# mahyarnajibi/SNIPER

Hardware: AMD Instinct MI355X
Metric: train chips/sec (512x512, R101) (higher is better)
Workload: dtype f16

## Files before the change

include/sniper_hip.h:

```cpp
#ifndef SNIPER_HIP_H
#define SNIPER_HIP_H

#include <stddef.h>
#include <stdint.h>

#ifdef __cplusplus
extern "C" {
#endif

typedef void *sn_stream_t;

enum { SN_OK = 0, SN_ERR_ARG = 1, SN_ERR_HIP = 2, SN_ERR_WORKSPACE = 3, SN_ERR_UNSUPPORTED = 4 };

int sn_version(void);
const char *sn_last_error(void);
int sn_debug_option(const char *name, int value);

int sn_iou_f64(const double *d_boxes, int N, const double *d_query, int K, double *d_out, int mode, sn_stream_t stream);

int sn_chips_num_candidates(int width, int height, int chipsize, int stride);
size_t sn_chips_workspace_bytes(int total_cand, int max_boxes_per_unit);
int sn_chips_generate_batch(const float *d_boxes, const int32_t *d_box_off, const int32_t *d_meta, const int32_t *d_perm,
                            const int32_t *d_cand_off, int U, int max_boxes_per_unit, void *d_mask_ws, float *d_out_chips,
                            int32_t *d_out_ids, int32_t *d_out_count, sn_stream_t stream);
// ... 74 lines not shown
                       int KH, int KWP, int stride, void *ws, size_t ws_bytes, sn_stream_t stream);
int sn_conv_dgrad(const void *dy, const void *wt, const void *accumulate, void *dx, int N, int H, int W, int Cin,
                  int dx_pix_stride, int Cout, int dy_pix_stride, int acc_pix_stride, int KH, int KW, int stride, int pad, int dil,
                  int out_f32, sn_stream_t stream);
int sn_conv_dgrad_by_class(int on);
int sn_conv_dgrad_bn_blocks(int N, int H, int W, int Cin, int dx_pix_stride, int Cout, int dy_pix_stride, int acc_pix_stride, int KH,
                            int KW, int stride, int pad, int dil);
int sn_conv_dgrad_bn(const void *dy, const void *wt, const void *accumulate, void *dx, int N, int H, int W, int Cin, int dx_pix_stride,
                     int Cout, int dy_pix_stride, int acc_pix_stride, int KH, int KW, int stride, int pad, int dil, const void *bn_x,
                     int bn_x_pix_stride, const float *bn_scale, const float *bn_shift, const float *bn_mean, int bn_act,
                     float *partials, sn_stream_t stream);
size_t sn_conv_wgrad_workspace_bytes(int N, int H, int W, int Cin, int x_pix_stride, int Cout, int dy_pix_stride, int KH, int KW,
                                     int stride, int pad, int dil);
int sn_conv_wgrad(const void *dy, const void *x, float *dw, int N, int H, int W, int Cin, int x_pix_stride, int Cout,
                  int dy_pix_stride, int KH, int KW, int stride, int pad, int dil, void *ws, size_t ws_bytes, sn_stream_t stream);
typedef struct sn_wgrad_desc {
  const void *dy, *x;
  float *dw;
  int N, H, W, Cin, x_pix_stride, Cout, dy_pix_stride, KH, KW, stride, pad, dil;
} sn_wgrad_desc;
size_t sn_conv_wgrad_batch_workspace_bytes(const sn_wgrad_desc *descs, int n);
int sn_conv_wgrad_batch(const sn_wgrad_desc *descs, int n, void *ws, size_t ws_bytes, sn_stream_t stream);
int sn_conv_wgrad_impl(int impl, int job_steps);
int sn_conv_wgrad_trace(void *buf);
int sn_conv_trace(void *buf);
size_t sn_bias_grad_workspace_bytes(long rows, int C);
int sn_bias_grad(const void *dy, float *db, long rows, int C, int ld, int dtype, void *ws, size_t ws_bytes, sn_stream_t stream);

int sn_pack_stem_input(const float *x_nchw, void *out, int N, int C, int H, int W, int Hp, int Wp, int pad_t, int pad_l,
                       const float *scale, const float *shift, sn_stream_t stream);

size_t sn_bn_workspace_bytes(int M, int C);
int sn_bn_stats(const void *x, int M, int C, int ps, void *ws, sn_stream_t stream);
int sn_bn_finalize(const void *ws, int M, int C, float eps, float momentum, const float *gamma, const float *beta,
                   float *run_mean, float *run_var, float *scale, float *shift, float *save_mean, float *save_invstd,
                   sn_stream_t stream);
int sn_bn_finalize_blocks(const float *partials, int nblk, int M, int C, float eps, float momentum, const float *gamma,
                          const float *beta, float *run_mean, float *run_var, float *scale, float *shift, float *save_mean,
                          float *save_invstd, sn_stream_t stream);
int sn_bn_global_scale_shift(const float *gamma, const float *beta, const float *mean, const float *var, int C, float eps,
                             float *scale, float *shift, sn_stream_t stream);
int sn_bn_apply(const void *x, void *y, int M, int C, int ps_in, int ps_out, const float *scale, const float *shift, int relu,
                sn_stream_t stream);
int sn_bn_apply_blocks(const float *partials, int nblk, const void *x, void *y, int M, int C, int ps_in, int ps_out, float eps,
                       float momentum, const float *gamma, const float *beta, float *run_mean, float *run_var, float *scale,
                       float *shift, float *save_mean, float *save_invstd, int relu, sn_stream_t stream);
// ... 110 lines not shown
```

sniper_amd/csrc/conv.hip:

```cpp
#include <algorithm>
#include <atomic>

#include "conv_common.h"

#include <stdlib.h>

__device__ __forceinline__ int swz(int row, int chunk) { return chunk ^ ((0x78 >> (2 * ((row >> 2) & 3))) & 3); }

template <int BM, int BN, bool DGRAD>
__global__ __launch_bounds__(256) void conv_igemm_kernel(const ConvParams p) {
  constexpr int BK = 32;
  constexpr int WM = BM / 2, WN = BN / 2;
  constexpr int MI = WM / 16, NI = WN / 16;
  constexpr int AR = BM / 64, BR = BN / 64;
  __shared__ __attribute__((aligned(16))) half_t sA[2][BM * BK];
  __shared__ __attribute__((aligned(16))) half_t sB[2][BN * BK];

  const int tid = threadIdx.x, lane = tid & 63, wave = tid >> 6;
  const int wm = wave >> 1, wn = wave & 1;
  const int m0 = blockIdx.x * BM, n0 = blockIdx.y * BN;
  const int chunk = tid & 3, lrow = tid >> 2;

  int a_base[AR], a_h[AR], a_w[AR];
  bool a_ok[AR];
// ... 624 lines not shown
  p.KH = KH; p.KW = KW; p.stride = stride; p.pad = pad; p.dil = dil;
  SN_REQUIRE(N > 0 && H > 0 && W > 0 && Cin > 0 && Cout > 0, "sn_conv_wgrad: bad dims");
  WgradPlan q = wgrad_plan(N, H, W, Cin, Cout, KH, KW, stride, pad, dil);
  p.Ho = q.Ho; p.Wo = q.Wo;
  SN_REQUIRE(p.Ho > 0 && p.Wo > 0, "sn_conv_wgrad: bad dims");
  const size_t n = (size_t)Cout * q.taps * Cin;
  p.slab = nullptr;
  p.slab_stride = n;
  if (q.splits > 1) {
    if (ws && ws_bytes >= sizeof(float) * (size_t)q.splits * n && ((uintptr_t)ws % 16) == 0) p.slab = (float *)ws;
    else { q.splits = 1; q.units_per_split = q.nunits; }
  }
  p.units_per_split = q.units_per_split;
  hipLaunchKernelGGL(conv_wgrad_kernel, dim3(wgrad_grid(p, q.gx, q.gy, q.taps * q.splits)), dim3(256), 0, s, p);
  SN_CHECK_LAUNCH();
  if (p.slab) {
    hipLaunchKernelGGL(wgrad_reduce_kernel, dim3(sn_blocks((long)(n / 4), 4096)), dim3(256), 0, s, (const float *)p.slab, q.splits, n, dw);
    SN_CHECK_LAUNCH();
  }
  return SN_OK;
}

static std::atomic<int> g_wgrad_na{0};
static std::atomic<int> g_wgrad_impl{1};
SN_EXPORT int sn_conv_wgrad_impl(int impl, int job_steps) {
  SN_REQUIRE((impl == 0 || impl == 1) && job_steps >= 0, "sn_conv_wgrad_impl: impl in {0, 1}, job_steps >= 0");
  SN_REQUIRE(job_steps / 100000 <= 2, "sn_conv_wgrad_impl: bad tile selector");
  g_wgrad_impl.store(impl, std::memory_order_relaxed);
  g_wgrad_na.store(job_steps / 100000, std::memory_order_relaxed);
  wgrad_ps_set_job_steps(job_steps % 100000);
  return SN_OK;
}

SN_EXPORT int sn_conv_trace(void *buf) {
  conv_dma_set_trace(static_cast<unsigned long long *>(buf));
  return SN_OK;
}

SN_EXPORT int sn_conv_wgrad_trace(void *buf) {
  wgrad_ps_set_trace(static_cast<unsigned long long *>(buf));
  return SN_OK;
}

static bool wgrad_desc_params(const sn_wgrad_desc &d, WgradParams &p) {
  p.dy = (const half_t *)d.dy; p.x = (const half_t *)d.x; p.dw = d.dw;
  p.N = d.N; p.H = d.H; p.W = d.W; p.Cin = d.Cin; p.Cout = d.Cout; p.dy_ps = d.dy_pix_stride; p.x_ps = d.x_pix_stride;
  p.KH = d.KH; p.KW = d.KW; p.stride = d.stride; p.pad = d.pad; p.dil = d.dil;
  if (d.N <= 0 || d.H <= 0 || d.W <= 0 || d.Cin <= 0 || d.Cout <= 0 || d.KH <= 0 || d.KW <= 0 || d.stride <= 0 || d.dil <= 0) return false;
  p.Ho = sn_conv_out(d.H, d.KH, d.stride, d.pad, d.dil);
  p.Wo = sn_conv_out(d.W, d.KW, d.stride, d.pad, d.dil);
  p.slab = nullptr; p.slab_stride = 0; p.units_per_split = 0;
  return p.Ho > 0 && p.Wo > 0;
}

static int wgrad_batch_run(const sn_wgrad_desc *descs, int n, void *ws, size_t ws_bytes, hipStream_t s, bool launch, size_t *need) {
  size_t off = 0;
  WgradParams chunk[kWgradMaxProblems];
  int nc = 0, na = 1;
  auto flush = [&]() -> int {
    if (!nc) return SN_OK;
    WgradBatch tab;
    char *base = ws ? static_cast<char *>(ws) + off : nullptr;
    size_t bytes = wgrad_ps_plan(chunk, nc, tab, base, true, na);
    if (launch) {
      if (bytes && !(ws && off + bytes <= ws_bytes && ((uintptr_t)base % 16) == 0)) bytes = wgrad_ps_plan(chunk, nc, tab, nullptr, false, na);
      if (int rc = wgrad_ps_launch(tab, s, na)) return rc;
    }
    off += bytes;
    nc = 0;
    return SN_OK;
  };
  for (int i = 0; i < n; ++i) {
    WgradParams p;
    SN_REQUIRE(wgrad_desc_params(descs[i], p), "sn_conv_wgrad_batch: bad dims in problem %d", i);
    if (launch) SN_REQUIRE(descs[i].dy && descs[i].x && descs[i].dw, "sn_conv_wgrad_batch: null pointer in problem %d", i);
  }
  auto fill = [](long j) { return j <= 0 ? 0.0 : (double)j / (256.0 * (double)((j + 255) / 256)); };
  for (int pass = 2; pass >= 1; --pass) {
    na = pass;
    long jobs = 0;
    for (int i = 0; i < n; ++i) {
      const sn_wgrad_desc &d = descs[i];
      WgradParams p;
      wgrad_desc_params(d, p);
      if (!(g_wgrad_impl.load(std::memory_order_relaxed) == 1 && wgrad_ps_ok(p))) continue;
      const int na_forced = g_wgrad_na.load(std::memory_order_relaxed);
      const int want = na_forced ? na_forced : (p.Cout > 128 ? 2 : 1);
      if (want != pass) continue;
      const bool flat = p.KH == 1 && p.KW == 1 && p.stride == 1 && p.pad == 0;
      const long steps = flat ? sn_div_up(sn_div_up(p.N * p.H * p.W, 32), 2) : sn_div_up(p.N * p.Ho * sn_div_up(p.Wo, 32), 2);
      const long j = (long)sn_div_up(p.Cout, 128 * na) * sn_div_up(p.Cin, 128) * p.KH * p.KW * ((steps + 399) / 400);
      if (nc && jobs >= 200 && fill(jobs) >= 0.93 && fill(jobs + j) < fill(jobs) - 0.02) {
        if (int rc = flush()) return rc;
        jobs = 0;
      }
      chunk[nc++] = p;
      jobs += j;
      if (nc == kWgradMaxProblems) {
        if (int rc = flush()) return rc;
        jobs = 0;
      }
    }
    if (int rc = flush()) return rc;
  }
  for (int i = 0; i < n; ++i) {
    const sn_wgrad_desc &d = descs[i];
    WgradParams p;
    wgrad_desc_params(d, p);
    if (g_wgrad_impl.load(std::memory_order_relaxed) == 1 && wgrad_ps_ok(p)) continue;
    const size_t bytes = wgrad_legacy_workspace_bytes(d.N, d.H, d.W, d.Cin, d.x_pix_stride, d.Cout, d.dy_pix_stride, d.KH, d.KW, d.stride, d.pad, d.dil);
    if (launch) {
      char *base = ws ? static_cast<char *>(ws) + off : nullptr;
      const size_t have = ws && off + bytes <= ws_bytes ? bytes : 0;
      if (int rc = wgrad_legacy(d.dy, d.x, d.dw, d.N, d.H, d.W, d.Cin, d.x_pix_stride, d.Cout, d.dy_pix_stride, d.KH, d.KW, d.stride, d.pad,
                                d.dil, have ? base : nullptr, have, s))
        return rc;
    }
    off += bytes;
  }
  if (need) *need = off;
  return SN_OK;
}

SN_EXPORT size_t sn_conv_wgrad_batch_workspace_bytes(const sn_wgrad_desc *descs, int n) {
  size_t need = 0;
  if (!descs || n <= 0 || wgrad_batch_run(descs, n, nullptr, 0, nullptr, false, &need)) return 0;
  return need;
}

SN_EXPORT int sn_conv_wgrad_batch(const sn_wgrad_desc *descs, int n, void *ws, size_t ws_bytes, sn_stream_t stream) {
  SN_REQUIRE(descs && n > 0, "sn_conv_wgrad_batch: empty table");
  return wgrad_batch_run(descs, n, ws, ws_bytes, sn_stream(stream), true, nullptr);
}

SN_EXPORT size_t sn_conv_wgrad_workspace_bytes(int N, int H, int W, int Cin, int x_pix_stride, int Cout, int dy_pix_stride, int KH,
                                               int KW, int stride, int pad, int dil) {
  const sn_wgrad_desc d = {nullptr, nullptr, nullptr, N, H, W, Cin, x_pix_stride, Cout, dy_pix_stride, KH, KW, stride, pad, dil};
  return sn_conv_wgrad_batch_workspace_bytes(&d, 1);
}

SN_EXPORT int sn_conv_wgrad(const void *dy, const void *x, float *dw, int N, int H, int W, int Cin, int x_pix_stride,
                            int Cout, int dy_pix_stride, int KH, int KW, int stride, int pad, int dil, void *ws,
                            size_t ws_bytes, sn_stream_t stream) {
// ... 49 lines not shown
```

sniper_amd/csrc/conv_common.h:

```cpp
#pragma once
#include <atomic>
#include "common.h"

struct ConvParams {
  const half_t *x;
  const half_t *w;
  void *y;
  const float *bias;
  const half_t *res;
  int N, H, W;
  int Cin, in_ps;
  int Ho, Wo;
  int Nout, out_ps, res_ps;
  int KH, KW, stride, pad, dil;
  int M;
  int relu, out_f32;
  unsigned x_bytes, w_bytes;
  const half_t *bn_x = nullptr;
  const float *bn_scale = nullptr, *bn_shift = nullptr, *bn_mean = nullptr;
  int bn_x_ps = 0, bn_act = 0;
  unsigned fda_mul = 1, fda_sh = 0, fdb_mul = 1, fdb_sh = 0;
  int rows_img = 1, row_len = 1;
  int cls = 0, cls_mc = 0;
  int ksplit = 1, ksplit_grid = 0;
// ... 70 lines not shown
  return true;
}
static inline unsigned wgrad_grid(WgradParams &p, int gx, int gy, int gz) {
  p.gx = gx; p.gy = gy; p.gz = gz;
  p.per_xcd = (gx * gy * gz + 7) / 8;
  return 8u * (unsigned)p.per_xcd;
}

struct WgradProblem {
  const half_t *dy, *x;
  float *dw, *slab;
  size_t slab_stride;
  int N, H, W, Ho, Wo, Cin, Cout, dy_ps, x_ps, KH, KW, stride, pad, dil;
  int gx, gy, taps, splits, units_per_split, cpr, nunits, item0;
};
constexpr int kWgradMaxProblems = 24;
struct WgradBatch {
  int n, total_items, per_xcd, reserved;
  int xcd_start[9];
  int reserved2;
  unsigned long long *trace;
  WgradProblem p[kWgradMaxProblems];
};
bool wgrad_ps_ok(const WgradParams &p);
size_t wgrad_ps_plan(const WgradParams *ps, int n, WgradBatch &tab, void *ws, bool allow_split, int na);
int wgrad_ps_launch(const WgradBatch &tab, hipStream_t s, int na);
void wgrad_ps_set_job_steps(int steps);
void wgrad_ps_set_trace(unsigned long long *buf);
```

sniper_amd/csrc/conv_wgrad_ps.hip:

```cpp
#include "conv_common.h"
#include <type_traits>

namespace {

constexpr int kTrSecond = 16 * 128;

constexpr unsigned kPoison = 0x80000000u;

constexpr int kTile = 64 * 128;

template <int S, int NA, int MI, bool TRACE>
__global__ __launch_bounds__(64 * (16 * NA / MI + 4)) void wgrad_ps_kernel(const WgradBatch tab) {
  constexpr int NI = 4, NC = 16 * NA / MI, L = 4 * (NA + 1);
  constexpr int kStage = (NA + 1) * kTile;
  static_assert((S - 1) * L < 64, "vmcnt is a 6-bit counter");
  __shared__ __attribute__((aligned(1024))) half_t lds[S * kStage];
  const int tid = threadIdx.x, lane = tid & 63;
  const int wave = __builtin_amdgcn_readfirstlane(tid >> 6);
  const unsigned long long t_entry = TRACE ? __builtin_amdgcn_s_memtime() : 0;
  const int b = blockIdx.x;
  const int item = tab.xcd_start[b & 7] + (b >> 3);
  if (item >= tab.xcd_start[(b & 7) + 1]) return;
  int pi = 0;
  while (pi + 1 < tab.n && item >= tab.p[pi + 1].item0) ++pi;
  const WgradProblem &P = tab.p[pi];
  const int gx = P.gx, taps = P.taps, tiles = gx * P.gy;
  int r = item - P.item0;
  const int bz = r / tiles;
  r -= bz * tiles;
  const int by = r / gx, bx = r - by * gx;
  const int split = bz / taps, tap = bz - split * taps;
  const int kh = tap / P.KW, kw = tap - kh * P.KW;
  const int co0 = bx * (128 * NA), ci0 = by * 128;
  const int Cout = P.Cout, Cin = P.Cin;
  const int u_begin = split * P.units_per_split, u_end = min(P.nunits, u_begin + P.units_per_split);
  const int nk = u_end > u_begin ? (u_end - u_begin + 1) >> 1 : 0;

  if (wave >= NC) {
    const int h = (wave - NC) >> 1, sub = (wave - NC) & 1;
    const int r4 = lane >> 4, slot = lane & 15;
    const unsigned dy_ps_b = (unsigned)P.dy_ps * 2u, x_ps_b = (unsigned)P.x_ps * 2u;
    const int stride = P.stride, Wo = P.Wo, Ho = P.Ho, H = P.H, W = P.W, cpr = P.cpr;
    const int row_shift = kh * P.dil - P.pad;
    unsigned a_base[NA][2], b_base[2];
#pragma unroll
    for (int o = 0; o < 2; ++o) {
      const int gc = ((((slot >> 1) ^ ((o << 2) | r4)) << 1) | (slot & 1));
      const int ur = 16 * sub + r4;
#pragma unroll
      for (int ta = 0; ta < NA; ++ta) {
// ... 32 lines not shown
          it_xc = 0;
          ++it_r;
          if (++it_oy == Ho) { it_oy = 0; ++it_img; }
        }
    };
#pragma unroll
    for (int s = 0; s < S - 1; ++s)
      if (s < nk) issue(s);
    int nxt = S - 1;
    unsigned long long c_wait = 0, c_bar = 0, c_issue = 0, t0 = 0, t1 = 0, t2 = 0;
    for (int t = 0; t < nk; ++t) {
      if (TRACE) t0 = __builtin_amdgcn_s_memtime();
      const int young = min(S - 2, nk - 1 - t);
      if (S > 3 && young >= 2) wait_vmcnt<(S > 3 ? 2 : 0) * L>();
      else if (S > 2 && young == 1) wait_vmcnt<(S > 2 ? 1 : 0) * L>();
      else wait_vmcnt<0>();
      if (TRACE) t1 = __builtin_amdgcn_s_memtime();
      __builtin_amdgcn_s_barrier();
      if (TRACE) t2 = __builtin_amdgcn_s_memtime();
      if (t + S - 1 < nk) issue(nxt);
      nxt = nxt + 1 == S ? 0 : nxt + 1;
      if (TRACE) { c_wait += t1 - t0; c_bar += t2 - t1; c_issue += __builtin_amdgcn_s_memtime() - t2; }
    }
    if (TRACE && wave == NC && lane == 0 && tab.trace) {
      unsigned long long *o = tab.trace + (size_t)item * 8;
      o[4] = c_wait; o[5] = c_bar; o[6] = c_issue;
    }
    return;
  }

  const int wm = wave >> 1, wn = wave & 1;
  const int fr = lane & 15, fq = lane >> 4;
  const int row0 = fq * 4 + (fr >> 2), q7 = row0 & 7;
  int a_off[MI], b_off[NI];
#pragma unroll
  for (int i = 0; i < MI; ++i) {
    const int rb = wm * MI + i;
    a_off[i] = (rb >> 3) * kTile + row0 * 128 + ((((rb & 7) ^ q7) << 4) | ((fr & 3) << 2));
  }
#pragma unroll
  for (int jn = 0; jn < NI; ++jn) b_off[jn] = row0 * 128 + ((((wn * 4 + jn) ^ q7) << 4) | ((fr & 3) << 2));
  floatx4 acc[MI][NI];
#pragma unroll
  for (int i = 0; i < MI; ++i)
#pragma unroll
    for (int jn = 0; jn < NI; ++jn) acc[i][jn] = floatx4{0.f, 0.f, 0.f, 0.f};
  unsigned long long c_bar = 0, tb = 0;
  const unsigned long long t_loop = TRACE ? __builtin_amdgcn_s_memtime() : 0;
// ... 29 lines not shown
  };
  if (nk > 0) {
    step_barrier();
    read(0, 0, fa0, fb0);
    __builtin_amdgcn_sched_barrier(0);
  }
  int cur = 0, nxt = 1;
  for (int t = 0; t + 1 < nk; ++t) {
    mma(fa0, fb0);
    read(cur, 1, fa1, fb1);
    interleave();
    step_barrier();
    __builtin_amdgcn_sched_barrier(0);
    mma(fa1, fb1);
    read(nxt, 0, fa0, fb0);
    interleave();
    cur = nxt;
    nxt = nxt + 1 == S ? 0 : nxt + 1;
  }
  if (nk > 0) {
    mma(fa0, fb0);
    read(cur, 1, fa1, fb1);
    interleave();
    mma(fa1, fb1);
  }
  const unsigned long long t_epi = TRACE ? __builtin_amdgcn_s_memtime() : 0;
  float *dst = P.slab ? P.slab + (size_t)split * P.slab_stride : P.dw;
  const bool to_slab = P.slab != nullptr;
  if ((Cin & 3) == 0) {
#pragma unroll
    for (int i0 = 0; i0 < MI; i0 += 4) {
      float *q[4][NI];
      bool ok[4][NI];
#pragma unroll
      for (int i = 0; i < 4; ++i)
#pragma unroll
        for (int jn = 0; jn < NI; ++jn) {
          const int co = co0 + (wm * MI + i0 + i) * 16 + fr, ci = ci0 + wn * 64 + jn * 16 + fq * 4;
          ok[i][jn] = co < Cout && ci < Cin;
          q[i][jn] = dst + ((size_t)co * taps + tap) * Cin + ci;
        }
      if (!to_slab) {
        float4 o[4][NI];
#pragma unroll
        for (int i = 0; i < 4; ++i)
#pragma unroll
          for (int jn = 0; jn < NI; ++jn) o[i][jn] = ok[i][jn] ? *reinterpret_cast<const float4 *>(q[i][jn]) : make_float4(0.f, 0.f, 0.f, 0.f);
#pragma unroll
// ... 5 lines not shown
          }
      }
#pragma unroll
      for (int i = 0; i < 4; ++i)
#pragma unroll
        for (int jn = 0; jn < NI; ++jn)
          if (ok[i][jn]) *reinterpret_cast<float4 *>(q[i][jn]) = make_float4(acc[i0 + i][jn][0], acc[i0 + i][jn][1], acc[i0 + i][jn][2], acc[i0 + i][jn][3]);
    }
  } else {
#pragma unroll
    for (int i = 0; i < MI; ++i) {
      const int co = co0 + (wm * MI + i) * 16 + fr;
      if (co >= Cout) continue;
#pragma unroll
      for (int jn = 0; jn < NI; ++jn) {
        const int ci = ci0 + wn * 64 + jn * 16 + fq * 4;
        float *qq = dst + ((size_t)co * taps + tap) * Cin + ci;
#pragma unroll
        for (int rr = 0; rr < 4; ++rr)
          if (ci + rr < Cin) qq[rr] = to_slab ? acc[i][jn][rr] : qq[rr] + acc[i][jn][rr];
      }
    }
  }
  if (TRACE && wave == 0 && lane == 0 && tab.trace) {
    asm volatile("s_waitcnt vmcnt(0)" ::: "memory");
    const unsigned long long t_end = __builtin_amdgcn_s_memtime();
    unsigned long long *o = tab.trace + (size_t)item * 8;
    o[0] = t_end - t_entry; o[1] = t_epi - t_loop; o[2] = c_bar; o[3] = t_end - t_epi; o[7] = (unsigned long long)nk;
  }
}

constexpr int kReduceBlocksMax = 1024;
__device__ __forceinline__ int reduce_blocks_of(const WgradProblem &q) {
  if (!q.slab) return 0;
  const long b = (long)((q.slab_stride / 4 + 255) / 256);
  return (int)(b < 1 ? 1 : (b > kReduceBlocksMax ? kReduceBlocksMax : b));
}
__global__ __launch_bounds__(256) void wgrad_reduce_batch_kernel(const WgradBatch tab) {
  int b = blockIdx.x, pi = 0, nb = 0;
  for (; pi < tab.n; ++pi) {
    nb = reduce_blocks_of(tab.p[pi]);
    if (b < nb) break;
    b -= nb;
  }
  if (pi >= tab.n) return;
  const WgradProblem &q = tab.p[pi];
  const float *__restrict__ slab = q.slab;
  float *__restrict__ dw = q.dw;
  const size_t n = q.slab_stride, n4 = n >> 2;
  const int splits = q.splits;
  for (size_t i = (size_t)b * 256 + threadIdx.x; i < n4; i += (size_t)nb * 256) {
    float4 a = reinterpret_cast<const float4 *>(dw)[i];
    int s = 0;
    for (; s + 8 <= splits; s += 8) {
      float4 v[8];
#pragma unroll
      for (int k = 0; k < 8; ++k) v[k] = reinterpret_cast<const float4 *>(slab + (size_t)(s + k) * n)[i];
#pragma unroll
      for (int k = 0; k < 8; ++k) { a.x += v[k].x; a.y += v[k].y; a.z += v[k].z; a.w += v[k].w; }
    }
    for (; s < splits; ++s) {
      const float4 v = reinterpret_cast<const float4 *>(slab + (size_t)s * n)[i];
      a.x += v.x; a.y += v.y; a.z += v.z; a.w += v.w;
    }
    reinterpret_cast<float4 *>(dw)[i] = a;
  }
  if (b == 0 && threadIdx.x < (n & 3)) {
    const size_t e = (n4 << 2) + threadIdx.x;
    float a = dw[e];
    for (int s = 0; s < splits; ++s) a += slab[(size_t)s * n + e];
    dw[e] = a;
  }
}

}

bool wgrad_ps_ok(const WgradParams &p) {
  const size_t xb = (size_t)p.N * p.H * p.W * p.x_ps * 2, dyb = (size_t)p.N * p.Ho * p.Wo * p.dy_ps * 2;
  return p.dy_ps % 8 == 0 && p.x_ps % 8 == 0 && p.dy_ps >= sn_div_up(p.Cout, 8) * 8 && p.x_ps >= sn_div_up(p.Cin, 8) * 8 &&
         ((uintptr_t)p.dy % 16) == 0 && ((uintptr_t)p.x % 16) == 0 && xb < (1ull << 30) && dyb < (1ull << 30) &&
         (size_t)p.Cout * p.KH * p.KW * p.Cin < (1ull << 31);
}

static std::atomic<unsigned long long *> g_wgrad_trace{nullptr};
void wgrad_ps_set_trace(unsigned long long *buf) { g_wgrad_trace.store(buf, std::memory_order_relaxed); }
static std::atomic<int> g_wgrad_job_steps{0};
void wgrad_ps_set_job_steps(int steps) { g_wgrad_job_steps.store(steps, std::memory_order_relaxed); }

size_t wgrad_ps_plan(const WgradParams *ps, int n, WgradBatch &tab, void *ws, bool allow_split, int na) {
  tab.n = n;
  long total_steps = 0;
  for (int i = 0; i < n; ++i) {
    const WgradParams &p = ps[i];
    WgradProblem &q = tab.p[i];
    q.dy = p.dy; q.x = p.x; q.dw = p.dw; q.slab = nullptr;
    const bool flat = p.KH == 1 && p.KW == 1 && p.stride == 1 && p.pad == 0;
    q.N = flat ? 1 : p.N; q.H = flat ? 1 : p.H; q.W = flat ? p.N * p.H * p.W : p.W;
    q.Ho = flat ? 1 : p.Ho; q.Wo = flat ? p.N * p.H * p.W : p.Wo;
    q.Cin = p.Cin; q.Cout = p.Cout; q.dy_ps = p.dy_ps; q.x_ps = p.x_ps;
    q.KH = p.KH; q.KW = p.KW; q.stride = p.stride; q.pad = p.pad; q.dil = p.dil;
    q.gx = sn_div_up(p.Cout, 128 * na); q.gy = sn_div_up(p.Cin, 128); q.taps = p.KH * p.KW;
    q.cpr = sn_div_up(q.Wo, 32);
    q.nunits = q.N * q.Ho * q.cpr;
    q.slab_stride = (size_t)p.Cout * q.taps * p.Cin;
    total_steps += (long)q.gx * q.gy * q.taps * sn_div_up(q.nunits, 2);
  }
  long cap = g_wgrad_job_steps.load(std::memory_order_relaxed);
  if (cap <= 0) {
    long longest = 1;
    for (int i = 0; i < n; ++i) { const long st = sn_div_up(tab.p[i].nunits, 2); longest = st > longest ? st : longest; }
    double best = 1e300;
    cap = longest;
    for (int sdiv = 1; sdiv <= 32; ++sdiv) {
      const long c = (longest + sdiv - 1) / sdiv;
      if (c < 16 && sdiv > 1) break;
      long jobs = 0;
      bool any_split = false;
      for (int i = 0; i < n; ++i) {
        const long st = sn_div_up(tab.p[i].nunits, 2), sp = (st + c - 1) / c;
        jobs += (long)tab.p[i].gx * tab.p[i].gy * tab.p[i].taps * sp;
        any_split |= sp > 1;
      }
      const double cost = (double)((jobs + 255) / 256) * (double)(c + 12) * (any_split ? 1.05 : 1.0);
      if (cost < best - 1e-9) { best = cost; cap = c; }
    }
    (void)total_steps;
  }
  if (!allow_split) cap = 1l << 30;
  size_t off = 0;
  int item = 0;
  for (int i = 0; i < n; ++i) {
    WgradProblem &q = tab.p[i];
    const int steps = sn_div_up(q.nunits, 2);
    int splits = sn_div_up(steps, (int)cap);
    if (splits < 1) splits = 1;
    int sps = sn_div_up(steps, splits);
    splits = sn_div_up(steps, sps);
    q.units_per_split = 2 * sps;
    q.splits = splits;
    if (splits > 1) {
      if (ws) q.slab = reinterpret_cast<float *>(static_cast<char *>(ws) + off);
      off += sn_align(sizeof(float) * (size_t)splits * q.slab_stride);
    }
    q.item0 = item;
    item += q.gx * q.gy * q.taps * splits;
  }
  tab.total_items = item;
  long work = 0;
  for (int i = 0; i < n; ++i) work += (long)(tab.p[i].units_per_split / 2) * tab.p[i].gx * tab.p[i].gy * tab.p[i].taps * tab.p[i].splits;
  {
    int x = 1, pi = 0, longest = 0;
    long done = 0;
    tab.xcd_start[0] = 0;
    for (int it = 0; it < item && x < 8; ++it) {
      while (pi + 1 < n && it >= tab.p[pi + 1].item0) ++pi;
      done += tab.p[pi].units_per_split / 2;
      if (done * 8 >= work * x) tab.xcd_start[x++] = it + 1;
    }
    for (; x <= 8; ++x) tab.xcd_start[x] = item;
    tab.xcd_start[8] = item;
    for (x = 0; x < 8; ++x) longest = tab.xcd_start[x + 1] - tab.xcd_start[x] > longest ? tab.xcd_start[x + 1] - tab.xcd_start[x] : longest;
    tab.per_xcd = longest;
  }
  tab.trace = g_wgrad_trace.load(std::memory_order_relaxed);
  return off;
}

int wgrad_ps_launch(const WgradBatch &tab, hipStream_t s, int na) {
  if (tab.total_items <= 0) return SN_OK;
  const dim3 grid(8u * (unsigned)tab.per_xcd);
  if (na == 2) {
    if (tab.trace) hipLaunchKernelGGL((wgrad_ps_kernel<3, 2, 4, true>), grid, dim3(768), 0, s, tab);
    else hipLaunchKernelGGL((wgrad_ps_kernel<3, 2, 4, false>), grid, dim3(768), 0, s, tab);
  } else {
    if (tab.trace) hipLaunchKernelGGL((wgrad_ps_kernel<4, 1, 4, true>), grid, dim3(512), 0, s, tab);
    else hipLaunchKernelGGL((wgrad_ps_kernel<4, 1, 4, false>), grid, dim3(512), 0, s, tab);
  }
  SN_CHECK_LAUNCH();
  long blocks = 0;
  for (int i = 0; i < tab.n; ++i) {
    const WgradProblem &q = tab.p[i];
    if (!q.slab) continue;
    const long b = (long)((q.slab_stride / 4 + 255) / 256);
    blocks += b < 1 ? 1 : (b > kReduceBlocksMax ? kReduceBlocksMax : b);
  }
  if (blocks > 0) {
    hipLaunchKernelGGL(wgrad_reduce_batch_kernel, dim3((unsigned)blocks), dim3(256), 0, s, tab);
    SN_CHECK_LAUNCH();
  }
  return SN_OK;
}
```

Before: 984.5.

## Add slot-balanced persistent wgrad scheduler with cached device-side job plans

```diff
diff --git a/include/sniper_hip.h b/include/sniper_hip.h
--- a/include/sniper_hip.h
+++ b/include/sniper_hip.h
@@ -120,6 +120,7 @@
 size_t sn_conv_wgrad_batch_workspace_bytes(const sn_wgrad_desc *descs, int n);
 int sn_conv_wgrad_batch(const sn_wgrad_desc *descs, int n, void *ws, size_t ws_bytes, sn_stream_t stream);
 int sn_conv_wgrad_impl(int impl, int job_steps);
+int sn_conv_wgrad_plan_stats(const sn_wgrad_desc *descs, int n, long *out);
 int sn_conv_wgrad_trace(void *buf);
 int sn_conv_trace(void *buf);
 size_t sn_bias_grad_workspace_bytes(long rows, int C);
diff --git a/sniper_amd/csrc/conv.hip b/sniper_amd/csrc/conv.hip
--- a/sniper_amd/csrc/conv.hip
+++ b/sniper_amd/csrc/conv.hip
@@ -1,5 +1,7 @@
+#include <string.h>
 #include <algorithm>
 #include <atomic>
+#include <vector>
 
 #include "conv_common.h"
 
@@ -670,9 +672,10 @@
 }
 
 static std::atomic<int> g_wgrad_na{0};
-static std::atomic<int> g_wgrad_impl{1};
+static int wgrad_impl_env() { const int v = sn_env_int("SNIPER_WGRAD_IMPL", 2); return v < 0 || v > 2 ? 2 : v; }
+static std::atomic<int> g_wgrad_impl{wgrad_impl_env()};
 SN_EXPORT int sn_conv_wgrad_impl(int impl, int job_steps) {
-  SN_REQUIRE((impl == 0 || impl == 1) && job_steps >= 0, "sn_conv_wgrad_impl: impl in {0, 1}, job_steps >= 0");
+  SN_REQUIRE(impl >= 0 && impl <= 2 && job_steps >= 0, "sn_conv_wgrad_impl: impl in {0, 1, 2}, job_steps >= 0");
   SN_REQUIRE(job_steps / 100000 <= 2, "sn_conv_wgrad_impl: bad tile selector");
   g_wgrad_impl.store(impl, std::memory_order_relaxed);
   g_wgrad_na.store(job_steps / 100000, std::memory_order_relaxed);
@@ -701,8 +704,14 @@
   return p.Ho > 0 && p.Wo > 0;
 }
 
-static int wgrad_batch_run(const sn_wgrad_desc *descs, int n, void *ws, size_t ws_bytes, hipStream_t s, bool launch, size_t *need) {
-  size_t off = 0;
+static int wgrad_class_of(const WgradParams &p) {
+  if (!(g_wgrad_impl.load(std::memory_order_relaxed) >= 1 && wgrad_ps_ok(p))) return 0;
+  const int na_forced = g_wgrad_na.load(std::memory_order_relaxed);
+  return na_forced ? na_forced : (p.Cout > 128 ? 2 : 1);
+}
+
+static int wgrad_batch_chunked(const sn_wgrad_desc *descs, int n, void *ws, size_t ws_bytes, hipStream_t s, bool launch, size_t *off_io) {
+  size_t off = *off_io;
   WgradParams chunk[kWgradMaxProblems];
   int nc = 0, na = 1;
   auto flush = [&]() -> int {
@@ -718,23 +727,14 @@
     nc = 0;
     return SN_OK;
   };
-  for (int i = 0; i < n; ++i) {
-    WgradParams p;
-    SN_REQUIRE(wgrad_desc_params(descs[i], p), "sn_conv_wgrad_batch: bad dims in problem %d", i);
-    if (launch) SN_REQUIRE(descs[i].dy && descs[i].x && descs[i].dw, "sn_conv_wgrad_batch: null pointer in problem %d", i);
-  }
   auto fill = [](long j) { return j <= 0 ? 0.0 : (double)j / (256.0 * (double)((j + 255) / 256)); };
   for (int pass = 2; pass >= 1; --pass) {
     na = pass;
     long jobs = 0;
     for (int i = 0; i < n; ++i) {
-      const sn_wgrad_desc &d = descs[i];
       WgradParams p;
-      wgrad_desc_params(d, p);
-      if (!(g_wgrad_impl.load(std::memory_order_relaxed) == 1 && wgrad_ps_ok(p))) continue;
-      const int na_forced = g_wgrad_na.load(std::memory_order_relaxed);
-      const int want = na_forced ? na_forced : (p.Cout > 128 ? 2 : 1);
-      if (want != pass) continue;
+      wgrad_desc_params(descs[i], p);
+      if (wgrad_class_of(p) != pass) continue;
       const bool flat = p.KH == 1 && p.KW == 1 && p.stride == 1 && p.pad == 0;
       const long steps = flat ? sn_div_up(sn_div_up(p.N * p.H * p.W, 32), 2) : sn_div_up(p.N * p.Ho * sn_div_up(p.Wo, 32), 2);
       const long j = (long)sn_div_up(p.Cout, 128 * na) * sn_div_up(p.Cin, 128) * p.KH * p.KW * ((steps + 399) / 400);
@@ -751,11 +751,57 @@
     }
     if (int rc = flush()) return rc;
   }
+  *off_io = off;
+  return SN_OK;
+}
+
+static void wgrad_split_classes(const sn_wgrad_desc *descs, int n, std::vector<WgradParams> cls[2]) {
+  for (int i = 0; i < n; ++i) {
+    WgradParams p;
+    wgrad_desc_params(descs[i], p);
+    const int c = wgrad_class_of(p);
+    if (c) cls[2 - c].push_back(p);
+  }
+}
+
+static int wgrad_batch_run(const sn_wgrad_desc *descs, int n, void *ws, size_t ws_bytes, hipStream_t s, bool launch, size_t *need) {
+  for (int i = 0; i < n; ++i) {
+    WgradParams p;
+    SN_REQUIRE(wgrad_desc_params(descs[i], p), "sn_conv_wgrad_batch: bad dims in problem %d", i);
+    if (launch) SN_REQUIRE(descs[i].dy && descs[i].x && descs[i].dw, "sn_conv_wgrad_batch: null pointer in problem %d", i);
+  }
+  size_t off = 0;
+  bool ran = false;
+  if (launch && g_wgrad_impl.load(std::memory_order_relaxed) == 2) {
+    if (int rc = wgrad_batch_chunked(descs, n, nullptr, 0, s, false, &off)) return rc;
+    std::vector<WgradParams> cls[2];
+    wgrad_split_classes(descs, n, cls);
+    if (!cls[0].empty() || !cls[1].empty()) {
+      const bool usable = ws && ((uintptr_t)ws % 16) == 0;
+      const size_t budget = usable ? std::min(off, ws_bytes) : 0;
+      std::vector<char> key(sizeof(sn_wgrad_desc) * (size_t)n + sizeof(int) * 2 + sizeof(void *) + sizeof(size_t));
+      char *k = key.data();
+      memcpy(k, descs, sizeof(sn_wgrad_desc) * (size_t)n); k += sizeof(sn_wgrad_desc) * (size_t)n;
+      const int na_forced = g_wgrad_na.load(std::memory_order_relaxed);
+      memcpy(k, &n, sizeof(int)); k += sizeof(int);
+      memcpy(k, &na_forced, sizeof(int)); k += sizeof(int);
+      memcpy(k, &ws, sizeof(void *)); k += sizeof(void *);
+      memcpy(k, &ws_bytes, sizeof(size_t));
+      if (int rc = wgrad_balanced_run(cls[0].data(), (int)cls[0].size(), cls[1].data(), (int)cls[1].size(), ws, budget, key.data(), key.size(), s, &ran))
+        return rc;
+    } else {
+      ran = true;
+    }
+  }
+  if (!ran) {
+    off = 0;
+    if (int rc = wgrad_batch_chunked(descs, n, ws, ws_bytes, s, launch, &off)) return rc;
+  }
   for (int i = 0; i < n; ++i) {
     const sn_wgrad_desc &d = descs[i];
     WgradParams p;
     wgrad_desc_params(d, p);
-    if (g_wgrad_impl.load(std::memory_order_relaxed) == 1 && wgrad_ps_ok(p)) continue;
+    if (wgrad_class_of(p)) continue;
     const size_t bytes = wgrad_legacy_workspace_bytes(d.N, d.H, d.W, d.Cin, d.x_pix_stride, d.Cout, d.dy_pix_stride, d.KH, d.KW, d.stride, d.pad, d.dil);
     if (launch) {
       char *base = ws ? static_cast<char *>(ws) + off : nullptr;
@@ -767,6 +813,29 @@
     off += bytes;
   }
   if (need) *need = off;
+  return SN_OK;
+}
+
+SN_EXPORT int sn_conv_wgrad_plan_stats(const sn_wgrad_desc *descs, int n, long *out) {
+  SN_REQUIRE(descs && n > 0 && out, "sn_conv_wgrad_plan_stats: empty table");
+  size_t need = 0;
+  if (int rc = wgrad_batch_run(descs, n, nullptr, 0, nullptr, false, &need)) return rc;
+  size_t budget = 0;
+  if (int rc = wgrad_batch_chunked(descs, n, nullptr, 0, nullptr, false, &budget)) return rc;
+  std::vector<WgradParams> cls[2];
+  wgrad_split_classes(descs, n, cls);
+  WgradClassStats st[2];
+  const size_t used = wgrad_balanced_stats(cls[0].data(), (int)cls[0].size(), cls[1].data(), (int)cls[1].size(), budget, st);
+  SN_REQUIRE(used <= budget, "sn_conv_wgrad_plan_stats: the plan's slabs exceed the scratch");
+  out[0] = (st[0].jobs > 0) + (st[1].jobs > 0);
+  out[1] = (st[0].reduce_blocks > 0) + (st[1].reduce_blocks > 0);
+  out[2] = (long)need;
+  for (int k = 0; k < 2; ++k) {
+    long *o = out + 3 + 6 * k;
+    o[0] = st[k].jobs; o[1] = st[k].jobs_listed; o[2] = st[k].jobs_distinct;
+    o[3] = st[k].ksteps; o[4] = st[k].heaviest_ksteps; o[5] = st[k].heaviest_cost;
+  }
+  out[15] = (long)used;
   return SN_OK;
 }
 
diff --git a/sniper_amd/csrc/conv_common.h b/sniper_amd/csrc/conv_common.h
--- a/sniper_amd/csrc/conv_common.h
+++ b/sniper_amd/csrc/conv_common.h
@@ -116,8 +116,23 @@
   unsigned long long *trace;
   WgradProblem p[kWgradMaxProblems];
 };
+constexpr int kWgradSlots = 256;
+struct WgradJob { int problem, r; };
+struct WgradReduceRange { int problem, block0, blocks, reserved; };
+struct WgradSlots {
+  const WgradProblem *p;
+  const int *slot_start;
+  const WgradJob *jobs;
+  const WgradReduceRange *red;
+  int n_red, reserved;
+  unsigned long long *trace;
+};
+struct WgradClassStats { long jobs, jobs_listed, jobs_distinct, ksteps, heaviest_ksteps, heaviest_cost; int reduce_blocks; };
 bool wgrad_ps_ok(const WgradParams &p);
 size_t wgrad_ps_plan(const WgradParams *ps, int n, WgradBatch &tab, void *ws, bool allow_split, int na);
 int wgrad_ps_launch(const WgradBatch &tab, hipStream_t s, int na);
+int wgrad_balanced_run(const WgradParams *ps2, int n2, const WgradParams *ps1, int n1, void *ws, size_t budget, const void *key,
+                       size_t key_bytes, hipStream_t s, bool *ran);
+size_t wgrad_balanced_stats(const WgradParams *ps2, int n2, const WgradParams *ps1, int n1, size_t budget, WgradClassStats stats[2]);
 void wgrad_ps_set_job_steps(int steps);
 void wgrad_ps_set_trace(unsigned long long *buf);
diff --git a/sniper_amd/csrc/conv_wgrad_ps.hip b/sniper_amd/csrc/conv_wgrad_ps.hip
--- a/sniper_amd/csrc/conv_wgrad_ps.hip
+++ b/sniper_amd/csrc/conv_wgrad_ps.hip
@@ -1,5 +1,9 @@
 #include "conv_common.h"
+#include <string.h>
+#include <algorithm>
+#include <mutex>
 #include <type_traits>
+#include <vector>
 
 namespace {
 
@@ -9,8 +13,8 @@
 
 constexpr int kTile = 64 * 128;
 
-template <int S, int NA, int MI, bool TRACE>
-__global__ __launch_bounds__(64 * (16 * NA / MI + 4)) void wgrad_ps_kernel(const WgradBatch tab) {
+template <int S, int NA, int MI, bool TRACE, bool MULTI>
+__device__ __forceinline__ void wgrad_ps_job(const WgradProblem &P, int r, unsigned long long *trace) {
   constexpr int NI = 4, NC = 16 * NA / MI, L = 4 * (NA + 1);
   constexpr int kStage = (NA + 1) * kTile;
   static_assert((S - 1) * L < 64, "vmcnt is a 6-bit counter");
@@ -18,14 +22,8 @@
   const int tid = threadIdx.x, lane = tid & 63;
   const int wave = __builtin_amdgcn_readfirstlane(tid >> 6);
   const unsigned long long t_entry = TRACE ? __builtin_amdgcn_s_memtime() : 0;
-  const int b = blockIdx.x;
-  const int item = tab.xcd_start[b & 7] + (b >> 3);
-  if (item >= tab.xcd_start[(b & 7) + 1]) return;
-  int pi = 0;
-  while (pi + 1 < tab.n && item >= tab.p[pi + 1].item0) ++pi;
-  const WgradProblem &P = tab.p[pi];
+  const int item = P.item0 + r;
   const int gx = P.gx, taps = P.taps, tiles = gx * P.gy;
-  int r = item - P.item0;
   const int bz = r / tiles;
   r -= bz * tiles;
   const int by = r / gx, bx = r - by * gx;
@@ -104,8 +102,9 @@
       nxt = nxt + 1 == S ? 0 : nxt + 1;
       if (TRACE) { c_wait += t1 - t0; c_bar += t2 - t1; c_issue += __builtin_amdgcn_s_memtime() - t2; }
     }
-    if (TRACE && wave == NC && lane == 0 && tab.trace) {
-      unsigned long long *o = tab.trace + (size_t)item * 8;
+    if (MULTI) __builtin_amdgcn_s_barrier();
+    if (TRACE && wave == NC && lane == 0 && trace) {
+      unsigned long long *o = trace + (size_t)item * 8;
       o[4] = c_wait; o[5] = c_bar; o[6] = c_issue;
     }
     return;
@@ -181,8 +180,12 @@
     mma(fa0, fb0);
     read(cur, 1, fa1, fb1);
     interleave();
-    mma(fa1, fb1);
-  }
+  }
+  if (MULTI) {
+    step_barrier();
+    __builtin_amdgcn_sched_barrier(0);
+  }
+  if (nk > 0) mma(fa1, fb1);
   const unsigned long long t_epi = TRACE ? __builtin_amdgcn_s_memtime() : 0;
   float *dst = P.slab ? P.slab + (size_t)split * P.slab_stride : P.dw;
   const bool to_slab = P.slab != nullptr;
@@ -234,29 +237,41 @@
       }
     }
   }
-  if (TRACE && wave == 0 && lane == 0 && tab.trace) {
+  if (TRACE && wave == 0 && lane == 0 && trace) {
     asm volatile("s_waitcnt vmcnt(0)" ::: "memory");
     const unsigned long long t_end = __builtin_amdgcn_s_memtime();
-    unsigned long long *o = tab.trace + (size_t)item * 8;
+    unsigned long long *o = trace + (size_t)item * 8;
     o[0] = t_end - t_entry; o[1] = t_epi - t_loop; o[2] = c_bar; o[3] = t_end - t_epi; o[7] = (unsigned long long)nk;
   }
 }
 
+template <int S, int NA, int MI, bool TRACE>
+__global__ __launch_bounds__(64 * (16 * NA / MI + 4)) void wgrad_ps_kernel(const WgradBatch tab) {
+  const int b = blockIdx.x;
+  const int item = tab.xcd_start[b & 7] + (b >> 3);
+  if (item >= tab.xcd_start[(b & 7) + 1]) return;
+  int pi = 0;
+  while (pi + 1 < tab.n && item >= tab.p[pi + 1].item0) ++pi;
+  wgrad_ps_job<S, NA, MI, TRACE, false>(tab.p[pi], item - tab.p[pi].item0, tab.trace);
+}
+
+template <int S, int NA, int MI, bool TRACE>
+__global__ __launch_bounds__(64 * (16 * NA / MI + 4)) void wgrad_ps_kernel_slots(const WgradSlots pl) {
+  const int b = blockIdx.x;
+  const int j0 = __builtin_amdgcn_readfirstlane(pl.slot_start[b]), j1 = __builtin_amdgcn_readfirstlane(pl.slot_start[b + 1]);
+  for (int j = j0; j < j1; ++j) {
+    const int pi = __builtin_amdgcn_readfirstlane(pl.jobs[j].problem), r = __builtin_amdgcn_readfirstlane(pl.jobs[j].r);
+    wgrad_ps_job<S, NA, MI, TRACE, true>(pl.p[pi], r, pl.trace);
+  }
+}
+
 constexpr int kReduceBlocksMax = 1024;
-__device__ __forceinline__ int reduce_blocks_of(const WgradProblem &q) {
-  if (!q.slab) return 0;
-  const long b = (long)((q.slab_stride / 4 + 255) / 256);
+__host__ __device__ inline int reduce_blocks_for(size_t slab_stride) {
+  const long b = (long)((slab_stride / 4 + 255) / 256);
   return (int)(b < 1 ? 1 : (b > kReduceBlocksMax ? kReduceBlocksMax : b));
 }
-__global__ __launch_bounds__(256) void wgrad_reduce_batch_kernel(const WgradBatch tab) {
-  int b = blockIdx.x, pi = 0, nb = 0;
-  for (; pi < tab.n; ++pi) {
-    nb = reduce_blocks_of(tab.p[pi]);
-    if (b < nb) break;
-    b -= nb;
-  }
-  if (pi >= tab.n) return;
-  const WgradProblem &q = tab.p[pi];
+__host__ __device__ inline int reduce_blocks_of(const WgradProblem &q) { return q.slab ? reduce_blocks_for(q.slab_stride) : 0; }
+__device__ __forceinline__ void wgrad_reduce_problem(const WgradProblem &q, int b, int nb) {
   const float *__restrict__ slab = q.slab;
   float *__restrict__ dw = q.dw;
   const size_t n = q.slab_stride, n4 = n >> 2;
@@ -284,6 +299,24 @@
     dw[e] = a;
   }
 }
+__global__ __launch_bounds__(256) void wgrad_reduce_batch_kernel(const WgradBatch tab) {
+  int b = blockIdx.x, pi = 0, nb = 0;
+  for (; pi < tab.n; ++pi) {
+    nb = reduce_blocks_of(tab.p[pi]);
+    if (b < nb) break;
+    b -= nb;
+  }
+  if (pi >= tab.n) return;
+  wgrad_reduce_problem(tab.p[pi], b, nb);
+}
+__global__ __launch_bounds__(256) void wgrad_reduce_slots_kernel(const WgradSlots pl) {
+  const int b = blockIdx.x;
+  int k = 0;
+  while (k + 1 < pl.n_red && b >= pl.red[k + 1].block0) ++k;
+  const WgradReduceRange rr = pl.red[k];
+  if (b - rr.block0 >= rr.blocks) return;
+  wgrad_reduce_problem(pl.p[rr.problem], b - rr.block0, rr.blocks);
+}
 
 }
 
@@ -299,50 +332,47 @@
 static std::atomic<int> g_wgrad_job_steps{0};
 void wgrad_ps_set_job_steps(int steps) { g_wgrad_job_steps.store(steps, std::memory_order_relaxed); }
 
-size_t wgrad_ps_plan(const WgradParams *ps, int n, WgradBatch &tab, void *ws, bool allow_split, int na) {
-  tab.n = n;
-  long total_steps = 0;
-  for (int i = 0; i < n; ++i) {
-    const WgradParams &p = ps[i];
-    WgradProblem &q = tab.p[i];
-    q.dy = p.dy; q.x = p.x; q.dw = p.dw; q.slab = nullptr;
-    const bool flat = p.KH == 1 && p.KW == 1 && p.stride == 1 && p.pad == 0;
-    q.N = flat ? 1 : p.N; q.H = flat ? 1 : p.H; q.W = flat ? p.N * p.H * p.W : p.W;
-    q.Ho = flat ? 1 : p.Ho; q.Wo = flat ? p.N * p.H * p.W : p.Wo;
-    q.Cin = p.Cin; q.Cout = p.Cout; q.dy_ps = p.dy_ps; q.x_ps = p.x_ps;
-    q.KH = p.KH; q.KW = p.KW; q.stride = p.stride; q.pad = p.pad; q.dil = p.dil;
-    q.gx = sn_div_up(p.Cout, 128 * na); q.gy = sn_div_up(p.Cin, 128); q.taps = p.KH * p.KW;
-    q.cpr = sn_div_up(q.Wo, 32);
-    q.nunits = q.N * q.Ho * q.cpr;
-    q.slab_stride = (size_t)p.Cout * q.taps * p.Cin;
-    total_steps += (long)q.gx * q.gy * q.taps * sn_div_up(q.nunits, 2);
-  }
+static void wgrad_problem_fill(const WgradParams &p, WgradProblem &q, int na) {
+  q.dy = p.dy; q.x = p.x; q.dw = p.dw; q.slab = nullptr;
+  const bool flat = p.KH == 1 && p.KW == 1 && p.stride == 1 && p.pad == 0;
+  q.N = flat ? 1 : p.N; q.H = flat ? 1 : p.H; q.W = flat ? p.N * p.H * p.W : p.W;
+  q.Ho = flat ? 1 : p.Ho; q.Wo = flat ? p.N * p.H * p.W : p.Wo;
+  q.Cin = p.Cin; q.Cout = p.Cout; q.dy_ps = p.dy_ps; q.x_ps = p.x_ps;
+  q.KH = p.KH; q.KW = p.KW; q.stride = p.stride; q.pad = p.pad; q.dil = p.dil;
+  q.gx = sn_div_up(p.Cout, 128 * na); q.gy = sn_div_up(p.Cin, 128); q.taps = p.KH * p.KW;
+  q.cpr = sn_div_up(q.Wo, 32);
+  q.nunits = q.N * q.Ho * q.cpr;
+  q.slab_stride = (size_t)p.Cout * q.taps * p.Cin;
+}
+
+static long wgrad_choose_cap(const WgradProblem *q, int n) {
   long cap = g_wgrad_job_steps.load(std::memory_order_relaxed);
-  if (cap <= 0) {
-    long longest = 1;
-    for (int i = 0; i < n; ++i) { const long st = sn_div_up(tab.p[i].nunits, 2); longest = st > longest ? st : longest; }
-    double best = 1e300;
-    cap = longest;
-    for (int sdiv = 1; sdiv <= 32; ++sdiv) {
-      const long c = (longest + sdiv - 1) / sdiv;
-      if (c < 16 && sdiv > 1) break;
-      long jobs = 0;
-      bool any_split = false;
-      for (int i = 0; i < n; ++i) {
-        const long st = sn_div_up(tab.p[i].nunits, 2), sp = (st + c - 1) / c;
-        jobs += (long)tab.p[i].gx * tab.p[i].gy * tab.p[i].taps * sp;
-        any_split |= sp > 1;
-      }
-      const double cost = (double)((jobs + 255) / 256) * (double)(c + 12) * (any_split ? 1.05 : 1.0);
-      if (cost < best - 1e-9) { best = cost; cap = c; }
-    }
-    (void)total_steps;
-  }
-  if (!allow_split) cap = 1l << 30;
+  if (cap > 0) return cap;
+  long longest = 1;
+  for (int i = 0; i < n; ++i) { const long st = sn_div_up(q[i].nunits, 2); longest = st > longest ? st : longest; }
+  double best = 1e300;
+  cap = longest;
+  for (int sdiv = 1; sdiv <= 32; ++sdiv) {
+    const long c = (longest + sdiv - 1) / sdiv;
+    if (c < 16 && sdiv > 1) break;
+    long jobs = 0;
+    bool any_split = false;
+    for (int i = 0; i < n; ++i) {
+      const long st = sn_div_up(q[i].nunits, 2), sp = (st + c - 1) / c;
+      jobs += (long)q[i].gx * q[i].gy * q[i].taps * sp;
+      any_split |= sp > 1;
+    }
+    const double cost = (double)((jobs + 255) / 256) * (double)(c + 12) * (any_split ? 1.05 : 1.0);
+    if (cost < best - 1e-9) { best = cost; cap = c; }
+  }
+  return cap;
+}
+
+static size_t wgrad_apply_cap(WgradProblem *qs, int n, long cap, void *ws, int *items) {
   size_t off = 0;
   int item = 0;
   for (int i = 0; i < n; ++i) {
-    WgradProblem &q = tab.p[i];
+    WgradProblem &q = qs[i];
     const int steps = sn_div_up(q.nunits, 2);
     int splits = sn_div_up(steps, (int)cap);
     if (splits < 1) splits = 1;
@@ -350,6 +380,7 @@
     splits = sn_div_up(steps, sps);
     q.units_per_split = 2 * sps;
     q.splits = splits;
+    q.slab = nullptr;
     if (splits > 1) {
       if (ws) q.slab = reinterpret_cast<float *>(static_cast<char *>(ws) + off);
       off += sn_align(sizeof(float) * (size_t)splits * q.slab_stride);
@@ -357,6 +388,17 @@
     q.item0 = item;
     item += q.gx * q.gy * q.taps * splits;
   }
+  *items = item;
+  return off;
+}
+
+size_t wgrad_ps_plan(const WgradParams *ps, int n, WgradBatch &tab, void *ws, bool allow_split, int na) {
+  tab.n = n;
+  for (int i = 0; i < n; ++i) wgrad_problem_fill(ps[i], tab.p[i], na);
+  long cap = wgrad_choose_cap(tab.p, n);
+  if (!allow_split) cap = 1l << 30;
+  int item = 0;
+  const size_t off = wgrad_apply_cap(tab.p, n, cap, ws, &item);
   tab.total_items = item;
   long work = 0;
   for (int i = 0; i < n; ++i) work += (long)(tab.p[i].units_per_split / 2) * tab.p[i].gx * tab.p[i].gy * tab.p[i].taps * tab.p[i].splits;
@@ -371,6 +413,10 @@
     }
     for (; x <= 8; ++x) tab.xcd_start[x] = item;
     tab.xcd_start[8] = item;
+    if (item <= kWgradSlots) {
+      for (x = 1; x < 8; ++x) tab.xcd_start[x] = std::min(tab.xcd_start[x], tab.xcd_start[x - 1] + 32);
+      for (x = 7; x >= 1; --x) tab.xcd_start[x] = std::max(tab.xcd_start[x], tab.xcd_start[x + 1] - 32);
+    }
     for (x = 0; x < 8; ++x) longest = tab.xcd_start[x + 1] - tab.xcd_start[x] > longest ? tab.xcd_start[x + 1] - tab.xcd_start[x] : longest;
     tab.per_xcd = longest;
   }
@@ -390,15 +436,254 @@
   }
   SN_CHECK_LAUNCH();
   long blocks = 0;
-  for (int i = 0; i < tab.n; ++i) {
-    const WgradProblem &q = tab.p[i];
-    if (!q.slab) continue;
-    const long b = (long)((q.slab_stride / 4 + 255) / 256);
-    blocks += b < 1 ? 1 : (b > kReduceBlocksMax ? kReduceBlocksMax : b);
-  }
+  for (int i = 0; i < tab.n; ++i) blocks += reduce_blocks_of(tab.p[i]);
   if (blocks > 0) {
     hipLaunchKernelGGL(wgrad_reduce_batch_kernel, dim3((unsigned)blocks), dim3(256), 0, s, tab);
     SN_CHECK_LAUNCH();
   }
   return SN_OK;
 }
+
+namespace {
+struct WgradClassPlan {
+  std::vector<WgradProblem> p;
+  std::vector<int> slot_start;
+  std::vector<WgradJob> jobs;
+  std::vector<WgradReduceRange> red;
+  int reduce_blocks = 0;
+  long cap = 0;
+  WgradClassStats st{};
+};
+
+int job_steps_of(const WgradProblem &q, int r) {
+  const int split = r / (q.gx * q.gy * q.taps);
+  const int u0 = split * q.units_per_split, u1 = std::min(q.nunits, u0 + q.units_per_split);
+  return u1 > u0 ? (u1 - u0 + 1) >> 1 : 0;
+}
+
+void wgrad_class_geometry(const WgradParams *ps, int n, int na, WgradClassPlan &c) {
+  c.p.resize(n);
+  for (int i = 0; i < n; ++i) wgrad_problem_fill(ps[i], c.p[i], na);
+  c.cap = n ? wgrad_choose_cap(c.p.data(), n) : 0;
+}
+
+void wgrad_class_assign(WgradClassPlan &c) {
+  const int n = (int)c.p.size();
+  struct J { int steps, problem, r; };
+  std::vector<J> js;
+  for (int i = 0; i < n; ++i) {
+    const WgradProblem &q = c.p[i];
+    const int cnt = q.gx * q.gy * q.taps * q.splits;
+    for (int r = 0; r < cnt; ++r) js.push_back({job_steps_of(q, r), i, r});
+  }
+  std::stable_sort(js.begin(), js.end(), [](const J &a, const J &b) { return a.steps > b.steps; });
+  std::vector<long> load(kWgradSlots, 0), steps(kWgradSlots, 0);
+  std::vector<std::vector<WgradJob>> lists(kWgradSlots);
+  std::vector<int> home(n, -1);
+  for (const J &j : js) {
+    long least = load[0];
+    for (int b = 1; b < kWgradSlots; ++b) least = std::min(least, load[b]);
+    int pick = -1;
+    if (home[j.problem] >= 0)
+      for (int b = home[j.problem]; b < kWgradSlots && pick < 0; b += 8)
+        if (load[b] == least) pick = b;
+    if (pick < 0) {
+      int best_x = 0, best_free = -1;
+      for (int x = 0; x < 8; ++x) {
+        int free_ = 0;
+        for (int b = x; b < kWgradSlots; b += 8) free_ += load[b] == least;
+        if (free_ > best_free) { best_free = free_; best_x = x; }
+      }
+      for (int b = best_x; b < kWgradSlots && pick < 0; b += 8)
+        if (load[b] == least) pick = b;
+    }
+    home[j.problem] = pick & 7;
+    load[pick] += j.steps + 12;
+    steps[pick] += j.steps;
+    lists[pick].push_back({j.problem, j.r});
+  }
+  c.slot_start.assign(kWgradSlots + 1, 0);
+  c.jobs.clear();
+  for (int b = 0; b < kWgradSlots; ++b) {
+    c.slot_start[b] = (int)c.jobs.size();
+    c.jobs.insert(c.jobs.end(), lists[b].begin(), lists[b].end());
+  }
+  c.slot_start[kWgradSlots] = (int)c.jobs.size();
+  c.red.clear();
+  c.reduce_blocks = 0;
+  for (int i = 0; i < n; ++i) {
+    if (c.p[i].splits <= 1) continue;
+    const int nb = reduce_blocks_for(c.p[i].slab_stride);
+    c.red.push_back({i, c.reduce_blocks, nb, 0});
+    c.reduce_blocks += nb;
+  }
+  WgradClassStats &st = c.st;
+  st = WgradClassStats{};
+  st.jobs = (long)js.size();
+  st.reduce_blocks = c.reduce_blocks;
+  std::vector<std::vector<char>> seen(n);
+  for (int i = 0; i < n; ++i) seen[i].assign((size_t)c.p[i].gx * c.p[i].gy * c.p[i].taps * c.p[i].splits, 0);
+  for (int b = 0; b < kWgradSlots; ++b) {
+    long cost = 0, ks = 0;
+    for (int k = c.slot_start[b]; k < c.slot_start[b + 1]; ++k) {
+      const WgradJob &j = c.jobs[k];
+      ++st.jobs_listed;
+      if (j.problem >= 0 && j.problem < n && j.r >= 0 && (size_t)j.r < seen[j.problem].size() && !seen[j.problem][j.r]) {
+        seen[j.problem][j.r] = 1;
+        ++st.jobs_distinct;
+        const int s_ = job_steps_of(c.p[j.problem], j.r);
+        ks += s_;
+        cost += s_ + 12;
+      }
+    }
+    st.ksteps += ks;
+    if (cost > st.heaviest_cost) { st.heaviest_cost = cost; st.heaviest_ksteps = ks; }
+  }
+}
+
+size_t wgrad_balanced_plan(const WgradParams *ps2, int n2, const WgradParams *ps1, int n1, void *ws, size_t budget, WgradClassPlan cls[2]) {
+  wgrad_class_geometry(ps2, n2, 2, cls[0]);
+  wgrad_class_geometry(ps1, n1, 1, cls[1]);
+  size_t bytes[2] = {0, 0};
+  int items = 0;
+  for (;;) {
+    for (int k = 0; k < 2; ++k) bytes[k] = cls[k].p.empty() ? 0 : wgrad_apply_cap(cls[k].p.data(), (int)cls[k].p.size(), cls[k].cap, nullptr, &items);
+    if (bytes[0] + bytes[1] <= budget) break;
+    WgradClassPlan &c = cls[bytes[0] >= bytes[1] ? 0 : 1];
+    c.cap = c.cap >= (1l << 28) ? (1l << 30) : c.cap + std::max(1l, c.cap / 8);
+  }
+  char *base = static_cast<char *>(ws);
+  for (int k = 0; k < 2; ++k) {
+    if (cls[k].p.empty()) { cls[k].slot_start.assign(kWgradSlots + 1, 0); continue; }
+    wgrad_apply_cap(cls[k].p.data(), (int)cls[k].p.size(), cls[k].cap, base && bytes[k] ? base + (k ? bytes[0] : 0) : nullptr, &items);
+    wgrad_class_assign(cls[k]);
+  }
+  return bytes[0] + bytes[1];
+}
+
+struct WgradCachedPlan {
+  std::vector<char> key;
+  void *dev = nullptr;
+  WgradSlots cls[2];
+  int jobs[2] = {0, 0}, reduce_blocks[2] = {0, 0};
+  unsigned long long used = 0;
+  bool pinned = false;
+};
+constexpr int kPlanCacheMax = 8;
+std::mutex g_plan_mu;
+std::vector<WgradCachedPlan> g_plans;
+unsigned long long g_plan_clock = 0;
+
+int wgrad_plan_upload(WgradClassPlan cls[2], WgradCachedPlan &e) {
+  size_t off[2][4], total = 0;
+  for (int k = 0; k < 2; ++k) {
+    const WgradClassPlan &c = cls[k];
+    const size_t sz[4] = {c.p.size() * sizeof(WgradProblem), c.slot_start.size() * sizeof(int), c.jobs.size() * sizeof(WgradJob),
+                          c.red.size() * sizeof(WgradReduceRange)};
+    for (int a = 0; a < 4; ++a) { off[k][a] = total; total += sn_align(sz[a] ? sz[a] : 1); }
+  }
+  std::vector<char> host(total, 0);
+  for (int k = 0; k < 2; ++k) {
+    const WgradClassPlan &c = cls[k];
+    if (!c.p.empty()) memcpy(host.data() + off[k][0], c.p.data(), c.p.size() * sizeof(WgradProblem));
+    memcpy(host.data() + off[k][1], c.slot_start.data(), c.slot_start.size() * sizeof(int));
+    if (!c.jobs.empty()) memcpy(host.data() + off[k][2], c.jobs.data(), c.jobs.size() * sizeof(WgradJob));
+    if (!c.red.empty()) memcpy(host.data() + off[k][3], c.red.data(), c.red.size() * sizeof(WgradReduceRange));
+  }
+  SN_HIP(hipMalloc(&e.dev, total));
+  if (hipError_t err = hipMemcpy(e.dev, host.data(), total, hipMemcpyHostToDevice)) {
+    (void)hipFree(e.dev);
+    e.dev = nullptr;
+    sn_set_error("wgrad plan upload: %s", hipGetErrorString(err));
+    return SN_ERR_HIP;
+  }
+  const char *d = static_cast<const char *>(e.dev);
+  for (int k = 0; k < 2; ++k) {
+    WgradSlots &t = e.cls[k];
+    t.p = reinterpret_cast<const WgradProblem *>(d + off[k][0]);
+    t.slot_start = reinterpret_cast<const int *>(d + off[k][1]);
+    t.jobs = reinterpret_cast<const WgradJob *>(d + off[k][2]);
+    t.red = reinterpret_cast<const WgradReduceRange *>(d + off[k][3]);
+    t.n_red = (int)cls[k].red.size();
+    t.reserved = 0;
+    t.trace = g_wgrad_trace.load(std::memory_order_relaxed);
+    e.jobs[k] = (int)cls[k].jobs.size();
+    e.reduce_blocks[k] = cls[k].reduce_blocks;
+  }
+  return SN_OK;
+}
+
+int wgrad_plan_launch(const WgradCachedPlan &e, hipStream_t s) {
+  const dim3 grid(kWgradSlots);
+  for (int k = 0; k < 2; ++k) {
+    if (!e.jobs[k]) continue;
+    const WgradSlots &t = e.cls[k];
+    if (k == 0) {
+      if (t.trace) hipLaunchKernelGGL((wgrad_ps_kernel_slots<3, 2, 4, true>), grid, dim3(768), 0, s, t);
+      else hipLaunchKernelGGL((wgrad_ps_kernel_slots<3, 2, 4, false>), grid, dim3(768), 0, s, t);
+    } else {
+      if (t.trace) hipLaunchKernelGGL((wgrad_ps_kernel_slots<4, 1, 4, true>), grid, dim3(512), 0, s, t);
+      else hipLaunchKernelGGL((wgrad_ps_kernel_slots<4, 1, 4, false>), grid, dim3(512), 0, s, t);
+    }
+    SN_CHECK_LAUNCH();
+    if (e.reduce_blocks[k] > 0) {
+      hipLaunchKernelGGL(wgrad_reduce_slots_kernel, dim3((unsigned)e.reduce_blocks[k]), dim3(256), 0, s, t);
+      SN_CHECK_LAUNCH();
+    }
+  }
+  return SN_OK;
+}
+}
+
+size_t wgrad_balanced_stats(const WgradParams *ps2, int n2, const WgradParams *ps1, int n1, size_t budget, WgradClassStats stats[2]) {
+  WgradClassPlan cls[2];
+  const size_t bytes = wgrad_balanced_plan(ps2, n2, ps1, n1, nullptr, budget, cls);
+  stats[0] = cls[0].st;
+  stats[1] = cls[1].st;
+  return bytes;
+}
+
+int wgrad_balanced_run(const WgradParams *ps2, int n2, const WgradParams *ps1, int n1, void *ws, size_t budget, const void *key,
+                       size_t key_bytes, hipStream_t s, bool *ran) {
+  *ran = false;
+  std::vector<char> k(key_bytes + sizeof(long) + sizeof(void *) + sizeof(int));
+  memcpy(k.data(), key, key_bytes);
+  const long steps = g_wgrad_job_steps.load(std::memory_order_relaxed);
+  unsigned long long *const tr = g_wgrad_trace.load(std::memory_order_relaxed);
+  int device = 0;
+  SN_HIP(hipGetDevice(&device));
+  memcpy(k.data() + key_bytes, &steps, sizeof(long));
+  memcpy(k.data() + key_bytes + sizeof(long), &tr, sizeof(void *));
+  memcpy(k.data() + key_bytes + sizeof(long) + sizeof(void *), &device, sizeof(int));
+  std::lock_guard<std::mutex> lock(g_plan_mu);
+  hipStreamCaptureStatus cap = hipStreamCaptureStatusNone;
+  SN_HIP(hipStreamIsCapturing(s, &cap));
+  const bool capturing = cap != hipStreamCaptureStatusNone;
+  WgradCachedPlan *hit = nullptr;
+  for (WgradCachedPlan &e : g_plans)
+    if (e.key.size() == k.size() && memcmp(e.key.data(), k.data(), k.size()) == 0) { hit = &e; break; }
+  if (!hit) {
+    if (capturing) return SN_OK;
+    WgradClassPlan cls[2];
+    wgrad_balanced_plan(ps2, n2, ps1, n1, ws, budget, cls);
+    int unpinned = 0, lru = -1;
+    for (int i = 0; i < (int)g_plans.size(); ++i)
+      if (!g_plans[i].pinned) {
+        ++unpinned;
+        if (lru < 0 || g_plans[i].used < g_plans[lru].used) lru = i;
+      }
+    if (unpinned >= kPlanCacheMax) {
+      SN_HIP(hipFree(g_plans[lru].dev));
+      g_plans.erase(g_plans.begin() + lru);
+    }
+    WgradCachedPlan e;
+    e.key = k;
+    if (int rc = wgrad_plan_upload(cls, e)) return rc;
+    g_plans.push_back(std::move(e));
+    hit = &g_plans.back();
+  }
+  hit->used = ++g_plan_clock;
+  hit->pinned |= capturing;
+  *ran = true;
+  return wgrad_plan_launch(*hit, s);
+}
```

Result: no change. 984.5 (-0.0%).
